# ybubnov/libhuffman

Hardware: AMD Instinct MI355X
Metric: encode+decode GiB/s (uncompressed) on 64KiB blocks (higher is better)
Workload: dtype u8; 1 GPU; configs[2]: 1 GiB Zipf-distributed bytes (zipf255 seed 3), blocksize=64KiB; generator=zipf255, bytes_per_gpu=1073741824, blocksize=65536, blocks_per_gpu=16384, compressed_bytes_per_gpu=1006904592, parallelism=block-sharded x1, bit_exact_roundtrip=True, decoder=sub-index (verified), one table pass per symbol

## Files before the change

libhuffman_amd/csrc/host/device.hpp:

```cpp
#pragma once

static SubStream sub_stream_args(const void *d_stream, uint64_t stream_len, const uint64_t *d_block_offsets, uint64_t nblocks,
                                 const void *d_sub_index, uint64_t raw_size, uint64_t blocksize, uint32_t flags)
{
    return {(const uint8_t *)d_stream, stream_len, d_block_offsets, nblocks, sub_index_view((void *)d_sub_index, raw_size, blocksize),
            raw_size, blocksize, max_tree_of(flags)};
}

extern "C" int hufgpu_fill(hufgpu_ctx_t *ctx, void *d_out, uint64_t n, int kind, uint64_t seed,
                           uint64_t first, void *stream)
{
    if (!ctx || (!d_out && n) || kind < 0 || kind > 3) return HUFE_ARGUMENT;
    if (n == 0) return HUFE_OK;
    if (kind == 1 && (first & 7)) {
        set_err(ctx, "uniform256 shards must start on an 8-byte boundary");
        return HUFE_ARGUMENT;
    }
    HIP_OK(ctx, hipSetDevice(ctx->device));
    hipStream_t s = pick_stream(ctx, stream);
    fill_kernel<<<dim3(4096), dim3(256), 0, s>>>((uint8_t *)d_out, n, kind, seed, first, ctx->d_zipf);
    HIP_OK(ctx, hipGetLastError());
    return HUFE_OK;
}

extern "C" int hufgpu_malloc(hufgpu_ctx_t *ctx, void **d_ptr, uint64_t bytes)
{
    if (!ctx || !d_ptr) return HUFE_ARGUMENT;
    HIP_OK(ctx, hipSetDevice(ctx->device));
    hipError_t e = hipMalloc(d_ptr, bytes ? bytes : 1);
    if (e != hipSuccess) {
        (void)hipGetLastError();
        set_err(ctx, "hipMalloc(%llu) failed: %s", (unsigned long long)bytes, hipGetErrorString(e));
        return HUFE_MEMORY;
    }
    return HUFE_OK;
}

extern "C" int hufgpu_free(hufgpu_ctx_t *ctx, void *d_ptr)
{
    if (!ctx) return HUFE_ARGUMENT;
    HIP_OK(ctx, hipSetDevice(ctx->device));
    HIP_OK(ctx, hipFree(d_ptr));
    return HUFE_OK;
}

extern "C" int hufgpu_memcpy_h2d(hufgpu_ctx_t *ctx, void *d_dst, const void *h_src, uint64_t bytes)
{
    if (!ctx) return HUFE_ARGUMENT;
    if (!bytes) return HUFE_OK;
    HIP_OK(ctx, hipSetDevice(ctx->device));
    HIP_OK(ctx, hipMemcpyAsync(d_dst, h_src, bytes, hipMemcpyHostToDevice, ctx->stream));
    HIP_OK(ctx, hipStreamSynchronize(ctx->stream));
    return HUFE_OK;
}

extern "C" int hufgpu_memcpy_d2h(hufgpu_ctx_t *ctx, void *h_dst, const void *d_src, uint64_t bytes)
{
    if (!ctx) return HUFE_ARGUMENT;
    if (!bytes) return HUFE_OK;
    HIP_OK(ctx, hipSetDevice(ctx->device));
    HIP_OK(ctx, hipMemcpyAsync(h_dst, d_src, bytes, hipMemcpyDeviceToHost, ctx->stream));
    HIP_OK(ctx, hipStreamSynchronize(ctx->stream));
    return HUFE_OK;
}

extern "C" int hufgpu_memcpy_d2d(hufgpu_ctx_t *ctx, void *d_dst, const void *d_src, uint64_t bytes)
{
    if (!ctx) return HUFE_ARGUMENT;
    if (!bytes) return HUFE_OK;
    HIP_OK(ctx, hipSetDevice(ctx->device));
    HIP_OK(ctx, hipMemcpyAsync(d_dst, d_src, bytes, hipMemcpyDeviceToDevice, ctx->stream));
    HIP_OK(ctx, hipStreamSynchronize(ctx->stream));
    return HUFE_OK;
}

extern "C" int hufgpu_synchronize(hufgpu_ctx_t *ctx)
{
    if (!ctx) return HUFE_ARGUMENT;
    HIP_OK(ctx, hipSetDevice(ctx->device));
    HIP_OK(ctx, hipStreamSynchronize(ctx->stream));
    return HUFE_OK;
}

template <int KIND>
static int calib_launch(int variant, const uint8_t *a, uint8_t *b, uint64_t bytes, uint32_t *flag, hipStream_t s)
{
#define CALIB_CASE(V, T, P, NTL, NTS) case V: calib_bw_kernel<T, P, KIND, NTL, NTS><<<dim3((unsigned)(bytes / P)), dim3(T), 0, s>>>(a, b, flag); return P;
    switch (variant) {
        CALIB_CASE(0, 256, 16384, true, true)
        CALIB_CASE(1, 256, 16384, true, false)
        CALIB_CASE(2, 256, 16384, false, false)
        CALIB_CASE(3, 512, 65536, true, true)
        CALIB_CASE(4, 512, 65536, true, false)
        CALIB_CASE(5, 256, 4096, true, true)
        CALIB_CASE(6, 256, 4096, false, false)
        CALIB_CASE(7, 1024, 65536, true, true)
    }
#undef CALIB_CASE
    return 0;
}
extern "C" int hufgpu_calib_bandwidth(hufgpu_ctx_t *ctx, int kind, int variant, const void *d_a, void *d_b, uint64_t bytes, void *stream)
{
    if (!ctx || kind < 0 || kind > 2 || variant < 0 || variant >= HUFGPU_CALIB_VARIANTS) return HUFE_ARGUMENT;
    if ((kind != 2 && !d_a) || (kind != 1 && !d_b) || bytes == 0 || (bytes & 65535u) || (((uintptr_t)d_a | (uintptr_t)d_b) & 15u)) return HUFE_ARGUMENT;
    HIP_OK(ctx, hipSetDevice(ctx->device));
    hipStream_t s = pick_stream(ctx, stream);
    uint32_t *flag = (uint32_t *)ctx->d_result;
    int per = 0;
    if (kind == 0) per = calib_launch<0>(variant, (const uint8_t *)d_a, (uint8_t *)d_b, bytes, flag + 6, s);
    else if (kind == 1) per = calib_launch<1>(variant, (const uint8_t *)d_a, (uint8_t *)d_b, bytes, flag + 6, s);
    else per = calib_launch<2>(variant, (const uint8_t *)d_a, (uint8_t *)d_b, bytes, flag + 6, s);
    HIP_OK(ctx, hipGetLastError());
    return per ? HUFE_OK : HUFE_ARGUMENT;
}

#ifdef DFAST_DEBUG
extern "C" int hufgpu_debug_dfast(unsigned long long *out32, int reset)
{
    if (reset) { unsigned long long z[DFAST_DBG_SLOTS] = {0}; return (int)hipMemcpyToSymbol(HIP_SYMBOL(hufgpu::g_dfast_dbg), z, sizeof(z)); }
    return (int)hipMemcpyFromSymbol(out32, HIP_SYMBOL(hufgpu::g_dfast_dbg), DFAST_DBG_SLOTS * sizeof(unsigned long long));
}
#endif
#ifdef TREE_DEBUG
extern "C" int hufgpu_debug_tree(unsigned long long *out, int reset)
{
    if (reset) { unsigned long long z[TREE_DBG_SLOTS] = {0}; return (int)hipMemcpyToSymbol(HIP_SYMBOL(hufgpu::g_tree_dbg), z, sizeof(z)); }
    return (int)hipMemcpyFromSymbol(out, HIP_SYMBOL(hufgpu::g_tree_dbg), TREE_DBG_SLOTS * sizeof(unsigned long long));
}
#endif

#ifdef DEC_PHASE_PROF
extern "C" int hufgpu_debug_phase_cycles(hufgpu_ctx_t *ctx, unsigned long long *out16, int reset)
{
    if (!ctx || !out16) return HUFE_ARGUMENT;
    HIP_OK(ctx, hipDeviceSynchronize());
    HIP_OK(ctx, hipMemcpyFromSymbol(out16, HIP_SYMBOL(hufgpu::g_dec_prof), 16 * sizeof(unsigned long long)));
    if (reset) {
        unsigned long long z[16] = {0};
        HIP_OK(ctx, hipMemcpyToSymbol(HIP_SYMBOL(hufgpu::g_dec_prof), z, sizeof(z)));
    }
    return HUFE_OK;
}
#endif
```

libhuffman_amd/csrc/kernels/pack.hpp:

```cpp
#pragma once
#include <hip/hip_runtime.h>
#include <stdint.h>

#include "../hufgpu_common.h"
#include "offsets.hpp"

namespace hufgpu {

#define PACK_SPT 32
#define PACK_STAGE_WORDS 3328

#define HUF_SUB_GROUP PACK_SPT
#define HUF_SUB_TILE  (64 * PACK_SPT)
struct HufSubIndex {
    uint64_t *tile_bits;
    uint16_t *group_bits;
    uint8_t *lens;
    uint64_t gpb, tpb;
};

template <typename CodeT>
struct PackAcc {
    uint64_t acc;
    uint32_t nacc;
    uint32_t first;
    bool have_first;
    uint32_t *gw;

    __device__ __forceinline__ void emit(uint32_t word)
    {
        if (!have_first) { first = word; have_first = true; }
        else *gw = __builtin_bswap32(word);
        gw++;
    }
    __device__ __forceinline__ void push32(uint32_t code, uint32_t len)
    {
        acc = (acc << len) | code;
        nacc += len;
        if (nacc >= 32) {
            nacc -= 32;
            emit((uint32_t)(acc >> nacc));
        }
    }
    __device__ __forceinline__ void push_pair(uint32_t e0, uint32_t e1)
    {
        const uint32_t l1 = e1 & 0xffu;
        push32(((e0 >> 8) << l1) | (e1 >> 8), (e0 & 0xffu) + l1);
    }
    __device__ __forceinline__ void push_triple(uint32_t e0, uint32_t e1, uint32_t e2)
    {
        const uint32_t l1 = e1 & 0xffu, l2 = e2 & 0xffu;
        push32(((((e0 >> 8) << l1) | (e1 >> 8)) << l2) | (e2 >> 8), (e0 & 0xffu) + l1 + l2);
    }
    __device__ __forceinline__ uint32_t tail() const { return (uint32_t)(acc & ((1ull << nacc) - 1ull)); }
    __device__ __forceinline__ void push(CodeT e)
    {
        uint32_t len = (uint32_t)(e & 0xffu);
        if constexpr (sizeof(CodeT) == 8) {
            const uint64_t c = e >> 8;
            if (len > 32) {
                push32((uint32_t)(c >> 32), len - 32);
                len = 32;
            }
            push32((uint32_t)c, len);
        } else {
            push32((uint32_t)(e >> 8), len);
        }
    }
};

#ifndef PACK_ACC64
template <>
struct PackAcc<uint32_t> {
    uint32_t acc;
    uint32_t nacc;
    uint32_t first;
    bool have_first;
    uint32_t *gw;

    __device__ __forceinline__ void emit(uint32_t word)
    {
        if (!have_first) { first = word; have_first = true; }
        else *gw = __builtin_bswap32(word);
        gw++;
    }
    __device__ __forceinline__ void push32(uint32_t code, uint32_t len)
    {
        const uint32_t out = acc >> ((32u - len) & 31u);
        acc = (acc << len) | code;
        nacc += len;
        if (nacc >= 32) {
            nacc -= 32;
            emit(__builtin_amdgcn_alignbit(out, acc, nacc));
        }
    }
    __device__ __forceinline__ void push_pair(uint32_t e0, uint32_t e1)
    {
        const uint32_t l1 = e1 & 0xffu;
        push32(((e0 >> 8) << l1) | (e1 >> 8), (e0 & 0xffu) + l1);
    }
    __device__ __forceinline__ void push_triple(uint32_t e0, uint32_t e1, uint32_t e2)
    {
        const uint32_t l1 = e1 & 0xffu, l2 = e2 & 0xffu;
        push32(((((e0 >> 8) << l1) | (e1 >> 8)) << l2) | (e2 >> 8), (e0 & 0xffu) + l1 + l2);
    }
    __device__ __forceinline__ void push(uint32_t e) { push32(e >> 8, e & 0xffu); }
    __device__ __forceinline__ uint32_t tail() const { return acc & ((1u << nacc) - 1u); }
};
#endif

__device__ __forceinline__ uint32_t header_byte(uint32_t j, uint64_t block_len, uint32_t tree_len,
                                                const int16_t *__restrict__ tb)
{
    if (j < 8) return (uint32_t)(block_len >> (8 * j)) & 0xffu;
    if (j < 10) return (tree_len >> (8 * (j - 8))) & 0xffu;
    const uint16_t e = (uint16_t)tb[(j - 10) >> 1];
    return (e >> (8 * (j & 1))) & 0xffu;
}

template <int THREADS>
__device__ __forceinline__ bool pack_header(uint64_t len, const int16_t *__restrict__ tb, uint32_t tree_len,
                                            uint8_t *g_a0, uint32_t *g_w0, uint32_t rec_lo, uint64_t rec_hi,
                                            uint32_t *s_tail, uint32_t *hdr_end_out)
{
    constexpr int WAVES = THREADS / 64;
    const int tid = (int)threadIdx.x;
    const uint32_t hdr_bytes = HUF_HEADER_FIXED + 2u * tree_len;
    const uint32_t hdr_end = rec_lo + hdr_bytes;
    for (uint32_t w = tid; w < (hdr_end >> 2); w += THREADS) {
        uint32_t v = 0;
#pragma unroll
        for (int k = 0; k < 4; k++) {
            const uint32_t bp = 4 * w + k;
            if (bp >= rec_lo) v |= header_byte(bp - rec_lo, len, tree_len, tb) << (8 * k);
        }
        if (4 * w >= rec_lo) g_w0[w] = v;
        else {
            for (uint32_t k = rec_lo - 4 * w; k < 4; k++) g_a0[4 * w + k] = (uint8_t)(v >> (8 * k));
        }
    }
    if (tree_len == 5) {
        for (uint32_t bp = (hdr_end & ~3u) + tid; bp < hdr_end; bp += THREADS)
            g_a0[bp] = (uint8_t)header_byte(bp - rec_lo, len, tree_len, tb);
        const uint64_t z0 = hdr_end, z1 = rec_hi;
        const uint64_t a0 = dmin<uint64_t>((z0 + 15) & ~15ull, z1);
        const uint64_t a1 = dmax<uint64_t>(a0, z1 & ~15ull);
        const uint64_t skew = (uint64_t)((uintptr_t)g_a0 & 15u);
        const uint64_t b0 = dmin<uint64_t>(((z0 + skew + 15) & ~15ull) - skew, z1);
        const uint64_t b1 = dmax<uint64_t>(b0, ((z1 + skew) & ~15ull) - skew);
        (void)a0; (void)a1;
        for (uint64_t bp = z0 + tid; bp < b0; bp += THREADS) g_a0[bp] = 0;
        uint4 *q = reinterpret_cast<uint4 *>(g_a0 + b0);
        const uint4 zero4 = make_uint4(0u, 0u, 0u, 0u);
        for (uint64_t i = (uint64_t)tid; i < ((b1 - b0) >> 4); i += THREADS) store_pack16(q + i, zero4);
        for (uint64_t bp = b1 + tid; bp < z1; bp += THREADS) g_a0[bp] = 0;
        return false;
    }
    if (tid == 0) {
        uint32_t t = 0;
        for (uint32_t bp = hdr_end & ~3u; bp < hdr_end; bp++)
            t = (t << 8) | header_byte(bp - rec_lo, len, tree_len, tb);
        s_tail[WAVES] = t;
    }
    __syncthreads();
    *hdr_end_out = hdr_end;
    return true;
}

template <int THREADS, typename CodeT, int GROUP = 1>
__device__ __forceinline__ void pack_block(const uint8_t *__restrict__ src, uint64_t len,
                                           const hufcode_t *__restrict__ codes64,
                                           const int16_t *__restrict__ tb, uint32_t tree_len,
                                           uint8_t *__restrict__ out, uint64_t dst0, uint64_t dst1,
                                           CodeT *s_code, uint32_t *s_part, uint32_t *s_tail, uint32_t *s_stage,
                                           uint64_t *__restrict__ sub_tiles, uint16_t *__restrict__ sub_groups)
{
    static_assert(HUF_SUB_TILE == 64 * PACK_SPT, "a sub-index tile is one wave of a pack tile");
    constexpr int TILE = THREADS * PACK_SPT;
    constexpr int WAVES = THREADS / 64;
    const int tid = (int)threadIdx.x;
    const int lane = tid & 63, wave = tid >> 6;

    uint8_t *g_a0 = out + (dst0 & ~3ull);
    const uint32_t rec_lo = (uint32_t)(dst0 & 3ull);
    const uint64_t rec_hi = rec_lo + (dst1 - dst0);
    uint32_t *g_w0 = reinterpret_cast<uint32_t *>(g_a0);

    for (int i = tid; i < HUF_NSYM; i += THREADS) s_code[i] = (CodeT)codes64[i];

    uint32_t hdr_end;
    if (!pack_header<THREADS>(len, tb, tree_len, g_a0, g_w0, rec_lo, rec_hi, s_tail, &hdr_end)) return;

    uint64_t bitpos = (uint64_t)hdr_end * 8ull;


    for (uint64_t t0 = 0; t0 < len; t0 += TILE) {
        const uint64_t my0 = t0 + (uint64_t)tid * PACK_SPT;
        uint32_t nsym = 0;
        CodeT code[PACK_SPT];
        uint32_t mybits = 0;
        if (my0 < len) {
            nsym = (uint32_t)dmin<uint64_t>(PACK_SPT, len - my0);
            const uint8_t *p = src + my0;
            if (nsym == PACK_SPT && (((uintptr_t)p) & 15u) == 0) {
                const uint4 v0 = load_stream16(reinterpret_cast<const uint4 *>(p));
                const uint4 v1 = load_stream16(reinterpret_cast<const uint4 *>(p) + 1);
                const uint32_t w[8] = {v0.x, v0.y, v0.z, v0.w, v1.x, v1.y, v1.z, v1.w};
#pragma unroll
                for (int k = 0; k < PACK_SPT; k++) code[k] = s_code[(w[k >> 2] >> (8 * (k & 3))) & 0xffu];
            } else {
#pragma unroll
                for (int k = 0; k < PACK_SPT; k++) code[k] = (k < (int)nsym) ? s_code[p[k]] : (CodeT)0;
            }
#pragma unroll
            for (int k = 0; k < PACK_SPT; k++) mybits += (uint32_t)(code[k] & 0xffu);
        } else {
#pragma unroll
            for (int k = 0; k < PACK_SPT; k++) code[k] = 0;
        }
        uint32_t tile_bits;
        const uint32_t ex = block_excl_scan_u32<THREADS>(mybits, s_part, tile_bits);
        if (sub_groups) {
            if (nsym) sub_groups[my0 / PACK_SPT] = (uint16_t)mybits;
            if (lane == 0 && nsym) sub_tiles[my0 / HUF_SUB_TILE] = bitpos + ex - (uint64_t)hdr_end * 8ull;
        }

        const uint64_t s = bitpos + ex;
        const uint64_t w_lo = bitpos >> 5, w_hi = (bitpos + tile_bits) >> 5;
        const uintptr_t stage_addr = (uintptr_t)(g_w0 + w_lo) & ~(uintptr_t)15;
        const uint32_t i_lo = (uint32_t)(((uintptr_t)(g_w0 + w_lo) - stage_addr) >> 2);
        const uint32_t i_hi = i_lo + (uint32_t)(w_hi - w_lo);
        const bool staged = i_hi + 2 <= PACK_STAGE_WORDS;
        PackAcc<CodeT> a;
        a.acc = 0;
        a.nacc = (uint32_t)(s & 31u);
        a.have_first = false;
        a.first = 0;
        uint32_t *const g_first = g_w0 + (s >> 5);
        uint32_t *const s_first = s_stage + (i_lo + (uint32_t)((s >> 5) - w_lo));
        if (staged) {
            a.gw = s_first;
            if constexpr (GROUP == 3) {
#pragma unroll
                for (int k = 0; k + 2 < PACK_SPT; k += 3) a.push_triple((uint32_t)code[k], (uint32_t)code[k + 1], (uint32_t)code[k + 2]);
                static_assert(PACK_SPT % 3 == 2, "the last two symbols go as a pair");
                a.push_pair((uint32_t)code[PACK_SPT - 2], (uint32_t)code[PACK_SPT - 1]);
            } else if constexpr (GROUP == 2) {
#pragma unroll
                for (int k = 0; k < PACK_SPT; k += 2) a.push_pair((uint32_t)code[k], (uint32_t)code[k + 1]);
            } else {
#pragma unroll
                for (int k = 0; k < PACK_SPT; k++) a.push(code[k]);
            }
        } else {
            a.gw = g_first;
#pragma unroll
            for (int k = 0; k < PACK_SPT; k++) a.push(code[k]);
        }
        const uint32_t nwords = (uint32_t)(a.gw - (staged ? s_first : g_first));
        const uint32_t tail_val = a.tail();

        uint32_t in_tail = wave_up1_u32(tail_val);
        if (lane == 63) s_tail[wave] = tail_val;
        __syncthreads();
        if (lane == 0) in_tail = (wave == 0) ? s_tail[WAVES] : s_tail[wave - 1];
        const uint32_t n_in = (uint32_t)(s & 31u);
        const bool is_last = (nsym > 0) && (my0 + nsym == len);
        if (a.have_first) {
            const uint32_t word = __builtin_bswap32(a.first | (n_in ? (in_tail << (32 - n_in)) : 0u));
            if (staged) *s_first = word;
            else *g_first = word;
        }
        uint32_t out_tail = tail_val;
        if (!a.have_first && nsym > 0) {
            out_tail = (n_in ? (in_tail << (a.nacc - n_in)) : 0u) | tail_val;
        }
        if (is_last && a.nacc) {
            const uint32_t word = out_tail << (32 - a.nacc);
            const uint32_t nbytes = (a.nacc + 7) >> 3;
            uint8_t *b = reinterpret_cast<uint8_t *>(g_first + nwords);
            for (uint32_t k = 0; k < nbytes; k++) b[k] = (uint8_t)(word >> (24 - 8 * k));
        }
        __syncthreads();
        if (tid == THREADS - 1) s_tail[WAVES] = out_tail;
        if (staged) {
            uint8_t *const g16 = reinterpret_cast<uint8_t *>(stage_addr);
            for (uint32_t u = tid; 4 * u < i_hi; u += THREADS) {
                const uint32_t i0 = 4 * u;
                if (i0 >= i_lo && i0 + 4 <= i_hi) {
                    store_pack16(reinterpret_cast<uint4 *>(g16 + 4 * i0), *reinterpret_cast<const uint4 *>(s_stage + i0));
                } else {
                    for (uint32_t i = (i0 > i_lo ? i0 : i_lo); i < i0 + 4 && i < i_hi; i++)
                        *reinterpret_cast<uint32_t *>(g16 + 4 * i) = s_stage[i];
                }
            }
        }
        bitpos += tile_bits;
        (void)rec_hi;
    }
}

struct PackEnt {
    uint32_t code;
    uint32_t lens;
};
__device__ __forceinline__ uint2 pack_ent_of(hufcode_t e)
{
    const uint32_t len = (uint32_t)(e & 0xffu);
    return make_uint2((uint32_t)(e >> 8), len | (((32u - len) & 31u) << 16) | (len << 27));
}
__device__ __forceinline__ uint32_t pack_pushed_out(uint32_t lens, uint32_t acc)
{
    uint32_t o;
    asm("v_lshrrev_b32_sdwa %0, %1, %2 dst_sel:DWORD dst_unused:UNUSED_PAD src0_sel:BYTE_2 src1_sel:DWORD"
        : "=v"(o) : "v"(lens), "v"(acc));
    return o;
}

template <int GROUP, bool PARTIAL>
__device__ __forceinline__ uint32_t pack_join(const uint2 *s_ent, const uint32_t (&w)[8], uint32_t nsym,
                                              uint32_t (&pc)[(PACK_SPT + GROUP - 1) / GROUP], uint32_t (&ph)[(PACK_SPT + GROUP - 1) / GROUP])
{
    constexpr int NG = (PACK_SPT + GROUP - 1) / GROUP;
    constexpr int BATCH = GROUP == 2 ? 4 : 2;
    uint32_t bits = 0;
#pragma unroll
    for (int g = 0; g < NG; g++) {
        if (g % BATCH == 0) __builtin_amdgcn_sched_barrier(0);
        const int k = g * GROUP;
        uint2 e[3];
#pragma unroll
        for (int j = 0; j < GROUP; j++) {
            const int kk = k + j;
            if (kk < PACK_SPT) {
                e[j] = s_ent[(w[kk >> 2] >> (8 * (kk & 3))) & 0xffu];
                if (PARTIAL && kk >= (int)nsym) e[j] = make_uint2(0u, 0u);
            }
        }
        if (GROUP == 3 && k + 2 < PACK_SPT) {
            pc[g] = (((e[0].x << (e[1].y & 31u)) | e[1].x) << (e[2].y & 31u)) | e[2].x;
            ph[g] = e[0].y + e[1].y + e[2].y;
        } else {
            pc[g] = (e[0].x << (e[1].y & 31u)) | e[1].x;
            ph[g] = e[0].y + e[1].y;
        }
        bits += ph[g];
    }
    __builtin_amdgcn_sched_barrier(0);
    return bits & 0xffffu;
}

template <int THREADS, int GROUP>
__device__ __forceinline__ void pack_block_multi(const uint8_t *__restrict__ src, uint64_t len64,
                                                 const hufcode_t *__restrict__ codes64,
                                                 const int16_t *__restrict__ tb, uint32_t tree_len,
                                                 uint8_t *__restrict__ out, uint64_t dst0, uint64_t dst1,
                                                 uint2 *s_ent, uint32_t *s_part, uint32_t *s_tail, uint32_t *s_stage,
                                                 uint64_t *__restrict__ sub_tiles, uint16_t *__restrict__ sub_groups)
{
    static_assert(GROUP == 2 || GROUP == 3, "two or three codes a push");
    static_assert(HUF_SUB_TILE == 64 * PACK_SPT, "a sub-index tile is one wave of a pack tile");
    constexpr uint32_t TILE = THREADS * PACK_SPT;
    constexpr int WAVES = THREADS / 64;
    const uint32_t len = (uint32_t)len64;
    constexpr int NG = (PACK_SPT + GROUP - 1) / GROUP;
    typedef __attribute__((address_space(3))) uint32_t *lds_word;
    const int tid = (int)threadIdx.x;
    const int lane = tid & 63, wave = tid >> 6;

    uint8_t *g_a0 = out + (dst0 & ~3ull);
    const uint32_t rec_lo = (uint32_t)(dst0 & 3ull);
    const uint64_t rec_hi = rec_lo + (dst1 - dst0);
    uint32_t *g_w0 = reinterpret_cast<uint32_t *>(g_a0);

    for (int i = tid; i < HUF_NSYM; i += THREADS) s_ent[i] = pack_ent_of(codes64[i]);

    uint32_t hdr_end;
    if (!pack_header<THREADS>(len64, tb, tree_len, g_a0, g_w0, rec_lo, rec_hi, s_tail, &hdr_end)) return;

    uint64_t bitpos = (uint64_t)hdr_end * 8ull;

    uint4 n0 = make_uint4(0u, 0u, 0u, 0u), n1 = n0;
    bool ahead = false;
#define PACK_REQUEST(T0_)                                                                                      \
    {                                                                                                         \
        const uint32_t m0_ = (T0_) + (uint32_t)tid * PACK_SPT;                                                \
        const uint8_t *q_ = src + m0_;                                                                        \
        ahead = (T0_) < len && __builtin_amdgcn_ballot_w64(!(m0_ + PACK_SPT <= len && (((uintptr_t)q_) & 15u) == 0)) == 0ull; \
        if (ahead) {                                                                                          \
            n0 = load_stream16(reinterpret_cast<const uint4 *>(q_));                                          \
            n1 = load_stream16(reinterpret_cast<const uint4 *>(q_) + 1);                                      \
        }                                                                                                     \
    }
    PACK_REQUEST(0u)
    for (uint32_t t0 = 0; t0 < len; t0 += TILE) {
        const uint32_t my0 = t0 + (uint32_t)tid * PACK_SPT;
        const uint32_t nsym = my0 < len ? dmin<uint32_t>(PACK_SPT, len - my0) : 0u;
        const uint8_t *p = src + my0;
        uint32_t pc[NG], ph[NG];
        uint32_t mybits;
        if (ahead) {
            const uint32_t w[8] = {n0.x, n0.y, n0.z, n0.w, n1.x, n1.y, n1.z, n1.w};
            mybits = pack_join<GROUP, false>(s_ent, w, nsym, pc, ph);
        } else {
            uint32_t w[8];
#pragma unroll
            for (int i = 0; i < 8; i++) {
                w[i] = 0;
#pragma unroll
                for (int j = 0; j < 4; j++)
                    if (4 * i + j < (int)nsym) w[i] |= (uint32_t)p[4 * i + j] << (8 * j);
            }
            mybits = pack_join<GROUP, true>(s_ent, w, nsym, pc, ph);
        }
        PACK_REQUEST(t0 + TILE)
        uint32_t tile_bits;
        const uint32_t ex = block_excl_scan_u32<THREADS>(mybits, s_part, tile_bits);
        if (sub_groups) {
            if (nsym) sub_groups[my0 / PACK_SPT] = (uint16_t)mybits;
            if (lane == 0 && nsym) sub_tiles[my0 / HUF_SUB_TILE] = bitpos + ex - (uint64_t)hdr_end * 8ull;
        }

        const uint64_t w_lo = bitpos >> 5, w_hi = (bitpos + tile_bits) >> 5;
        const uintptr_t stage_addr = (uintptr_t)(g_w0 + w_lo) & ~(uintptr_t)15;
        const uint32_t i_lo = (uint32_t)(((uintptr_t)(g_w0 + w_lo) - stage_addr) >> 2);
        const uint32_t i_hi = i_lo + (uint32_t)(w_hi - w_lo);
        const bool staged = i_hi + 2 <= PACK_STAGE_WORDS;
        const uint32_t rel = (uint32_t)(bitpos & 31u) + ex;
        const uint32_t n_in = rel & 31u;
        uint32_t *const g_first = g_w0 + w_lo + (rel >> 5);
        uint32_t *const s_first = s_stage + (i_lo + (rel >> 5));
        uint32_t nwords, nacc, tail_val, first = 0;
        if (staged) {
            uint32_t acc = 0;
            uint32_t tot = n_in | (n_in << 27);
            const uint32_t gw0 = (uint32_t)(uintptr_t)(lds_word)s_first - 4u;
            uint32_t gw = gw0;
#pragma unroll
            for (int g = 0; g < NG; g++) {
                uint32_t tot2;
                const bool word_done = __builtin_add_overflow(tot, ph[g], &tot2);
                const uint32_t acc2 = (acc << (ph[g] & 31u)) | pc[g];
                if (word_done) {
                    const uint32_t word = __builtin_amdgcn_alignbit(pack_pushed_out(ph[g], acc), acc2, tot2);
                    gw += 4;
                    asm volatile("" : "+v"(gw));
                    *(lds_word)(uintptr_t)gw = __builtin_bswap32(word);
                }
                acc = acc2;
                tot = tot2;
            }
            nwords = (gw - gw0) >> 2;
            nacc = tot & 31u;
            tail_val = acc & ((1u << nacc) - 1u);
        } else {
            PackAcc<uint32_t> a;
            a.acc = 0;
            a.nacc = n_in;
            a.have_first = false;
            a.first = 0;
            a.gw = g_first;
#pragma unroll 1
            for (uint32_t k = 0; k < nsym; k++) {
                const uint2 e = s_ent[src[my0 + k]];
                a.push32(e.x, e.y & 31u);
            }
            nwords = (uint32_t)(a.gw - g_first);
            nacc = a.nacc;
            tail_val = a.tail();
            first = a.first;
        }

        uint32_t in_tail = wave_up1_u32(tail_val);
        if (lane == 63) s_tail[wave] = tail_val;
        __syncthreads();
        if (lane == 0) in_tail = (wave == 0) ? s_tail[WAVES] : s_tail[wave - 1];
        const bool is_last = (nsym > 0) && (my0 + nsym == len);
        if (nwords) {
            const uint32_t lead = n_in ? (in_tail << (32 - n_in)) : 0u;
            if (staged) {
                if (n_in) __hip_atomic_fetch_or(s_first, __builtin_bswap32(lead), __ATOMIC_RELAXED, __HIP_MEMORY_SCOPE_WORKGROUP);
            } else {
                *g_first = __builtin_bswap32(first | lead);
            }
        }
        uint32_t out_tail = tail_val;
        if (!nwords && nsym > 0) {
            out_tail = (n_in ? (in_tail << (nacc - n_in)) : 0u) | tail_val;
        }
        if (is_last && nacc) {
            const uint32_t word = out_tail << (32 - nacc);
            const uint32_t nbytes = (nacc + 7) >> 3;
            uint8_t *b = reinterpret_cast<uint8_t *>(g_first + nwords);
            for (uint32_t k = 0; k < nbytes; k++) b[k] = (uint8_t)(word >> (24 - 8 * k));
        }
        __syncthreads();
        if (tid == THREADS - 1) s_tail[WAVES] = out_tail;
        if (staged) {
            uint8_t *const g16 = reinterpret_cast<uint8_t *>(stage_addr);
            for (uint32_t u = tid; 4 * u < i_hi; u += THREADS) {
                const uint32_t i0 = 4 * u;
                if (i0 >= i_lo && i0 + 4 <= i_hi) {
                    store_pack16(reinterpret_cast<uint4 *>(g16 + 4 * i0), *reinterpret_cast<const uint4 *>(s_stage + i0));
                } else {
                    for (uint32_t i = (i0 > i_lo ? i0 : i_lo); i < i0 + 4 && i < i_hi; i++)
                        *reinterpret_cast<uint32_t *>(g16 + 4 * i) = s_stage[i];
                }
            }
        }
        bitpos += tile_bits;
        (void)rec_hi;
    }
}

#undef PACK_REQUEST

template <int THREADS, bool SHORT>
__device__ __forceinline__ void pack_block_any(const uint8_t *__restrict__ src, uint64_t len, uint64_t row, uint64_t blk,
                                               const hufcode_t *__restrict__ codetab,
                                               const int16_t *__restrict__ treebuf,
                                               const HufBlockMeta *__restrict__ meta,
                                               uint64_t *__restrict__ offsets, const TwoLevel &sizes,
                                               uint8_t *__restrict__ out, const HufSubIndex &sub,
                                               hufcode_t *s_code, uint32_t *s_part, uint32_t *s_tail, uint32_t *s_stage)
{
    const HufBlockMeta m = meta[row];
    const hufcode_t *codes = codetab + row * HUF_NSYM;
    const int16_t *tb = treebuf + row * HUF_TREE_STRIDE;
    uint64_t o0, o1;
    if (sizes.local) {
        o0 = sizes.gprefix[blk / SCAN_GROUP] + sizes.local[blk];
        o1 = o0 + encoded_block_bytes(m);
        if (threadIdx.x == 0) offsets[blk] = o0;
    } else {
        o0 = offsets[blk];
        o1 = offsets[blk + 1];
    }
    uint64_t *sub_tiles = sub.tile_bits ? sub.tile_bits + blk * sub.tpb : nullptr;
    uint16_t *sub_groups = sub.tile_bits ? sub.group_bits + blk * sub.gpb : nullptr;
    if (sub.tile_bits && m.tree_len != 5)
        for (int i = (int)threadIdx.x; i < HUF_NSYM; i += THREADS) sub.lens[blk * HUF_NSYM + i] = (uint8_t)(codes[i] & 0xffu);
#if !defined(PACK_ACC64)
    if (m.max_len <= 10)
        pack_block_multi<THREADS, 3>(src, len, codes, tb, m.tree_len, out, o0, o1,
                                     reinterpret_cast<uint2 *>(s_code), s_part, s_tail, s_stage, sub_tiles, sub_groups);
    else if (m.max_len <= 15)
        pack_block_multi<THREADS, 2>(src, len, codes, tb, m.tree_len, out, o0, o1,
                                     reinterpret_cast<uint2 *>(s_code), s_part, s_tail, s_stage, sub_tiles, sub_groups);
#else
    if (m.max_len <= 10)
        pack_block<THREADS, uint32_t, 3>(src, len, codes, tb, m.tree_len, out, o0, o1,
                                         reinterpret_cast<uint32_t *>(s_code), s_part, s_tail, s_stage, sub_tiles, sub_groups);
    else if (m.max_len <= 15)
        pack_block<THREADS, uint32_t, 2>(src, len, codes, tb, m.tree_len, out, o0, o1,
                                            reinterpret_cast<uint32_t *>(s_code), s_part, s_tail, s_stage, sub_tiles, sub_groups);
#endif
    else if (SHORT || m.max_len <= 24)
        pack_block<THREADS, uint32_t>(src, len, codes, tb, m.tree_len, out, o0, o1,
                                      reinterpret_cast<uint32_t *>(s_code), s_part, s_tail, s_stage, sub_tiles, sub_groups);
    else if constexpr (!SHORT)
        pack_block<THREADS, hufcode_t>(src, len, codes, tb, m.tree_len, out, o0, o1,
                                       s_code, s_part, s_tail, s_stage, sub_tiles, sub_groups);
}

template <int THREADS, bool SHORT>
__device__ __forceinline__ void pack_block_any(const uint8_t *__restrict__ src, uint64_t len, uint64_t blk,
                                               const hufcode_t *__restrict__ codetab,
                                               const int16_t *__restrict__ treebuf,
                                               const HufBlockMeta *__restrict__ meta,
                                               uint64_t *__restrict__ offsets, const TwoLevel &sizes,
                                               uint8_t *__restrict__ out, const HufSubIndex &sub,
                                               hufcode_t *s_code, uint32_t *s_part, uint32_t *s_tail, uint32_t *s_stage)
{
    pack_block_any<THREADS, SHORT>(src, len, blk, blk, codetab, treebuf, meta, offsets, sizes, out, sub, s_code, s_part, s_tail, s_stage);
}

#ifndef PACK_WAVES_PER_SIMD
#define PACK_WAVES_PER_SIMD 6
#endif
template <int THREADS, bool SHORT>
__global__ __launch_bounds__(THREADS, SHORT ? PACK_WAVES_PER_SIMD : 4) void pack_kernel(const uint8_t *__restrict__ in, uint64_t n,
                                                       uint64_t blocksize,
                                                       const hufcode_t *__restrict__ codetab,
                                                       const int16_t *__restrict__ treebuf,
                                                       const HufBlockMeta *__restrict__ meta,
                                                       uint64_t *__restrict__ offsets, TwoLevel sizes,
                                                       uint8_t *__restrict__ out, HufSubIndex sub)
{
    __shared__ hufcode_t s_code[HUF_NSYM];
    __shared__ uint32_t s_part[THREADS / 64];
    __shared__ uint32_t s_tail[THREADS / 64 + 1];
    __shared__ __attribute__((aligned(16))) uint32_t s_stage[PACK_STAGE_WORDS];

#ifdef PACK_VGPR_SLACK
    asm volatile("; one VGPR more than the kernel uses" ::: PACK_VGPR_SLACK);
#endif
    const uint64_t blk = blockIdx.x;
    const uint64_t base = blk * blocksize;
    const uint64_t len = dmin<uint64_t>(blocksize, n - base);
    pack_block_any<THREADS, SHORT>(in + base, len, blk, codetab, treebuf, meta, offsets, sizes, out, sub,
                                   s_code, s_part, s_tail, s_stage);
}

}
```

libhuffman_amd/csrc/kernels/util.hpp:

```cpp
#pragma once
#include <hip/hip_runtime.h>
#include <stdint.h>

#include "../hufgpu_common.h"

namespace hufgpu {

__device__ __forceinline__ int lane_id() { return (int)(threadIdx.x & 63u); }

__device__ __forceinline__ uint32_t uni32(uint32_t v) { return (uint32_t)__builtin_amdgcn_readfirstlane((int)v); }
__device__ __forceinline__ uint64_t uni64(uint64_t v)
{
    return ((uint64_t)uni32((uint32_t)(v >> 32)) << 32) | uni32((uint32_t)v);
}
__device__ __forceinline__ void pin_uniform(uint64_t v)
{
    asm volatile("" :: "s"((uint32_t)v), "s"((uint32_t)(v >> 32)));
}

template <typename T>
__device__ __forceinline__ T dmin(T a, T b) { return a < b ? a : b; }
template <typename T>
__device__ __forceinline__ T dmax(T a, T b) { return a > b ? a : b; }

__device__ __forceinline__ uint64_t encoded_block_bytes(const HufBlockMeta &m)
{
    return (uint64_t)HUF_HEADER_FIXED + 2ull * m.tree_len + ((m.payload_bits + 7) >> 3);
}

__device__ __forceinline__ uint4 load_stream16(const uint4 *p)
{
    typedef uint32_t v4u __attribute__((ext_vector_type(4)));
    const v4u v = __builtin_nontemporal_load(reinterpret_cast<const v4u *>(p));
    return make_uint4(v.x, v.y, v.z, v.w);
}
__device__ __forceinline__ void store_stream16(uint4 *p, uint4 v)
{
    typedef uint32_t v4u __attribute__((ext_vector_type(4)));
    v4u t; t.x = v.x; t.y = v.y; t.z = v.z; t.w = v.w;
    __builtin_nontemporal_store(t, reinterpret_cast<v4u *>(p));
}
__device__ __forceinline__ void store_pack16(uint4 *p, uint4 v)
{
    *p = v;
}

__device__ __forceinline__ uint32_t wave_xor_any(uint32_t v, int o);
__device__ __forceinline__ uint64_t shfl_xor_u64(uint64_t v, int mask)
{
    return ((uint64_t)wave_xor_any((uint32_t)(v >> 32), mask) << 32) | wave_xor_any((uint32_t)v, mask);
}
__device__ __forceinline__ uint32_t shfl_xor_key(uint32_t v, int mask) { return (uint32_t)__shfl_xor((int)v, mask); }
__device__ __forceinline__ uint64_t shfl_xor_key(uint64_t v, int mask) { return shfl_xor_u64(v, mask); }

__device__ __forceinline__ uint32_t wave_incl_scan_u32(uint32_t v)
{
    v += (uint32_t)__builtin_amdgcn_update_dpp(0, (int)v, 0x111, 0xf, 0xf, true);
    v += (uint32_t)__builtin_amdgcn_update_dpp(0, (int)v, 0x112, 0xf, 0xf, true);
    v += (uint32_t)__builtin_amdgcn_update_dpp(0, (int)v, 0x114, 0xf, 0xf, true);
    v += (uint32_t)__builtin_amdgcn_update_dpp(0, (int)v, 0x118, 0xf, 0xf, true);
    v += (uint32_t)__builtin_amdgcn_update_dpp(0, (int)v, 0x142, 0xa, 0xf, false);
    v += (uint32_t)__builtin_amdgcn_update_dpp(0, (int)v, 0x143, 0xc, 0xf, false);
    return v;
}
__device__ __forceinline__ uint32_t wave_excl_max_u32(uint32_t v)
{
#define HUF_MAX_DPP_(ctrl, rmask, bc) { const uint32_t o_ = (uint32_t)__builtin_amdgcn_update_dpp(0, (int)v, ctrl, rmask, 0xf, bc); v = v > o_ ? v : o_; }
    HUF_MAX_DPP_(0x111, 0xf, true)
    HUF_MAX_DPP_(0x112, 0xf, true)
    HUF_MAX_DPP_(0x114, 0xf, true)
    HUF_MAX_DPP_(0x118, 0xf, true)
    HUF_MAX_DPP_(0x142, 0xa, false)
    HUF_MAX_DPP_(0x143, 0xc, false)
#undef HUF_MAX_DPP_
    return (uint32_t)__builtin_amdgcn_update_dpp(0, (int)v, 0x138, 0xf, 0xf, true);
}
__device__ __forceinline__ uint32_t pk_max_u16(uint32_t a, uint32_t b)
{
    typedef unsigned short us2 __attribute__((ext_vector_type(2)));
    const us2 r = __builtin_elementwise_max(__builtin_bit_cast(us2, a), __builtin_bit_cast(us2, b));
    return __builtin_bit_cast(uint32_t, r);
}

template <int D>
__device__ __forceinline__ uint32_t wave_xor_u32(uint32_t v)
{
    if constexpr (D == 1) return (uint32_t)__builtin_amdgcn_update_dpp(0, (int)v, 0xB1, 0xf, 0xf, false);
    else if constexpr (D == 2) return (uint32_t)__builtin_amdgcn_update_dpp(0, (int)v, 0x4E, 0xf, 0xf, false);
    else if constexpr (D == 4) {
        const uint32_t a = (uint32_t)__builtin_amdgcn_update_dpp(0, (int)v, 0x124, 0xf, 0xf, false);
        const uint32_t b = (uint32_t)__builtin_amdgcn_update_dpp(0, (int)v, 0x12C, 0xf, 0xf, false);
        return (lane_id() & 4) ? a : b;
    } else if constexpr (D == 8) return (uint32_t)__builtin_amdgcn_update_dpp(0, (int)v, 0x128, 0xf, 0xf, false);
    else if constexpr (D == 16) return (uint32_t)__builtin_amdgcn_ds_swizzle((int)v, 0x401F);
    else return (uint32_t)__shfl_xor((int)v, D);
}

__device__ __forceinline__ uint32_t wave_xor_any(uint32_t v, int o)
{
    return o == 1 ? wave_xor_u32<1>(v) : o == 2 ? wave_xor_u32<2>(v) : o == 4 ? wave_xor_u32<4>(v)
         : o == 8 ? wave_xor_u32<8>(v) : o == 16 ? wave_xor_u32<16>(v) : wave_xor_u32<32>(v);
}
__device__ __forceinline__ uint32_t wave_up1_u32(uint32_t v)
{
    return (uint32_t)__builtin_amdgcn_update_dpp((int)v, (int)v, 0x138, 0xf, 0xf, false);
}

__device__ __forceinline__ uint32_t wave_lane_u32(uint32_t v, uint32_t uniform_lane)
{
    return (uint32_t)__builtin_amdgcn_readlane((int)v, (int)uniform_lane);
}

template <int THREADS>
__device__ __forceinline__ uint32_t block_excl_scan_u32(uint32_t v, uint32_t *s_part, uint32_t &total)
{
    const int lane = lane_id();
    const int wave = (int)(threadIdx.x >> 6);
    const uint32_t inc = wave_incl_scan_u32(v);
    if (lane == 63) s_part[wave] = inc;
    __syncthreads();
    uint32_t base = 0, tot = 0;
#pragma unroll
    for (int i = 0; i < THREADS / 64; i++) {
        const uint32_t x = s_part[i];
        if (i < wave) base += x;
        tot += x;
    }
    __syncthreads();
    total = tot;
    return base + inc - v;
}

template <int THREADS, typename T>
__device__ __forceinline__ T block_excl_scan(T v, T *s_part, T &total)
{
    const int lane = lane_id();
    const int wave = (int)(threadIdx.x >> 6);
    T inc = v;
#pragma unroll
    for (int o = 1; o < 64; o <<= 1) {
        T t;
        if constexpr (sizeof(T) == 8) {
            uint32_t lo = (uint32_t)inc, hi = (uint32_t)((uint64_t)inc >> 32);
            lo = (uint32_t)__shfl_up((int)lo, o);
            hi = (uint32_t)__shfl_up((int)hi, o);
            t = (T)(((uint64_t)hi << 32) | lo);
        } else {
            t = (T)__shfl_up((int)inc, o);
        }
        if (lane >= o) inc += t;
    }
    if (lane == 63) s_part[wave] = inc;
    __syncthreads();
    T base = 0, tot = 0;
#pragma unroll
    for (int i = 0; i < THREADS / 64; i++) {
        T x = s_part[i];
        if (i < wave) base += x;
        tot += x;
    }
    __syncthreads();
    total = tot;
    return base + inc - v;
}

}
```

Baseline: 878.0 GiB/s.

## Overlap pack prologue loads: batch metadata scalar loads, prefetch codes/tree, vectorize header

Restructures the encode pack prologue. Per-block metadata and offsets are fetched with grouped scalar loads behind a single wait. Each thread loads its code-table entry and tree dwords up front, and the first input tile is requested before the header is written. The header is then built from registers with alignbit word stores instead of byte-wise loops, and the lens-row write is folded into the same pass. This aims to cut serialized memory latency at block start; the cost is more complex rec_lo alignment logic. It also adds optional cycle-profiling hooks that are compiled out by default.

```diff
diff --git a/libhuffman_amd/csrc/host/device.hpp b/libhuffman_amd/csrc/host/device.hpp
--- a/libhuffman_amd/csrc/host/device.hpp
+++ b/libhuffman_amd/csrc/host/device.hpp
@@ -129,6 +129,20 @@
 }
 #endif
 
+#ifdef PACK_PHASE_PROF
+extern "C" int hufgpu_debug_pack_phase_cycles(hufgpu_ctx_t *ctx, unsigned long long *out16, int reset)
+{
+    if (!ctx || !out16) return HUFE_ARGUMENT;
+    HIP_OK(ctx, hipDeviceSynchronize());
+    HIP_OK(ctx, hipMemcpyFromSymbol(out16, HIP_SYMBOL(hufgpu::g_pack_prof), 16 * sizeof(unsigned long long)));
+    if (reset) {
+        unsigned long long z[16] = {0};
+        HIP_OK(ctx, hipMemcpyToSymbol(HIP_SYMBOL(hufgpu::g_pack_prof), z, sizeof(z)));
+    }
+    return HUFE_OK;
+}
+#endif
+
 #ifdef DEC_PHASE_PROF
 extern "C" int hufgpu_debug_phase_cycles(hufgpu_ctx_t *ctx, unsigned long long *out16, int reset)
 {
diff --git a/libhuffman_amd/csrc/kernels/pack.hpp b/libhuffman_amd/csrc/kernels/pack.hpp
--- a/libhuffman_amd/csrc/kernels/pack.hpp
+++ b/libhuffman_amd/csrc/kernels/pack.hpp
@@ -118,37 +118,88 @@
     return (e >> (8 * (j & 1))) & 0xffu;
 }
 
+#ifdef PACK_PHASE_PROF
+__device__ unsigned long long g_pack_prof[16];
+#define PPROF_T() (__builtin_readcyclecounter())
+#define PPROF_ADD(slot, t0) do { if (threadIdx.x == 0) atomicAdd(&g_pack_prof[slot], (unsigned long long)(__builtin_readcyclecounter() - (t0))); } while (0)
+#define PPROF_WAIT() asm volatile("s_waitcnt vmcnt(0)" ::: "memory")
+#else
+#define PPROF_T() 0ull
+#define PPROF_ADD(slot, t0) do { (void)(t0); } while (0)
+#define PPROF_WAIT() do { } while (0)
+#endif
+
+#define PACK_TREE_DWORDS (HUF_TREE_STRIDE / 2)
+struct PackPre {
+    hufcode_t code;
+    uint32_t t[4];
+};
 template <int THREADS>
-__device__ __forceinline__ bool pack_header(uint64_t len, const int16_t *__restrict__ tb, uint32_t tree_len,
+__device__ __forceinline__ PackPre pack_pre_request(const hufcode_t *__restrict__ codes64, const int16_t *__restrict__ tb, uint32_t tid)
+{
+    static_assert(THREADS == HUF_NSYM, "one code-table entry a thread");
+    static_assert(3 * THREADS >= PACK_TREE_DWORDS && HUF_TREE_STRIDE % 4 == 0, "three tree dwords a thread cover an aligned row");
+    static_assert(2 * HUF_TREE_MAX <= 4 * (PACK_TREE_DWORDS - 1), "the look-ahead dword of the tree's last bytes is inside the row");
+    const uint32_t *tw = reinterpret_cast<const uint32_t *>(tb);
+    PackPre p;
+    p.code = codes64[tid];
+#pragma unroll
+    for (uint32_t k = 0; k < 4; k++) p.t[k] = tw[dmin<uint32_t>(3u * tid + k, PACK_TREE_DWORDS - 1u)];
+    return p;
+}
+
+__device__ __forceinline__ void pack_pre_arrived(const PackPre &p)
+{
+    asm volatile("" :: "v"((uint32_t)p.code), "v"((uint32_t)(p.code >> 32)), "v"(p.t[0]), "v"(p.t[1]), "v"(p.t[2]), "v"(p.t[3]));
+    __builtin_amdgcn_sched_barrier(0);
+}
+
+template <int THREADS>
+__device__ __forceinline__ bool pack_header(uint64_t len, const PackPre &pre, uint32_t tree_len,
                                             uint8_t *g_a0, uint32_t *g_w0, uint32_t rec_lo, uint64_t rec_hi,
-                                            uint32_t *s_tail, uint32_t *hdr_end_out)
+                                            uint32_t *s_tail, uint32_t *hdr_end_out, uint32_t tid)
 {
     constexpr int WAVES = THREADS / 64;
-    const int tid = (int)threadIdx.x;
     const uint32_t hdr_bytes = HUF_HEADER_FIXED + 2u * tree_len;
     const uint32_t hdr_end = rec_lo + hdr_bytes;
-    for (uint32_t w = tid; w < (hdr_end >> 2); w += THREADS) {
-        uint32_t v = 0;
-#pragma unroll
-        for (int k = 0; k < 4; k++) {
-            const uint32_t bp = 4 * w + k;
-            if (bp >= rec_lo) v |= header_byte(bp - rec_lo, len, tree_len, tb) << (8 * k);
-        }
-        if (4 * w >= rec_lo) g_w0[w] = v;
+    const uint32_t nwhole = hdr_end >> 2, nb = hdr_end & 3u;
+    const uint32_t wq0 = 3u + (rec_lo == 3u ? 1u : 0u);
+    const uint32_t cut = (8u * (2u - rec_lo)) & 31u;
+    if (tid == 0) {
+        const uint32_t f[4] = {(uint32_t)len, (uint32_t)(len >> 32), (tree_len & 0xffffu) | (pre.t[0] << 16), (pre.t[0] >> 16) | (pre.t[1] << 16)};
+        const uint32_t up = (32u - 8u * rec_lo) & 31u;
+        uint32_t v[4];
+        v[0] = f[0] << (8u * rec_lo);
+#pragma unroll
+        for (int w = 1; w < 4; w++) v[w] = rec_lo ? __builtin_amdgcn_alignbit(f[w], f[w - 1], up) : f[w];
+        if (rec_lo == 0) g_w0[0] = v[0];
         else {
-            for (uint32_t k = rec_lo - 4 * w; k < 4; k++) g_a0[4 * w + k] = (uint8_t)(v >> (8 * k));
+#pragma unroll
+            for (uint32_t k = 1; k < 4; k++)
+                if (k >= rec_lo) g_a0[k] = (uint8_t)(v[0] >> (8 * k));
+        }
+        g_w0[1] = v[1];
+        g_w0[2] = v[2];
+        if (rec_lo == 3) g_w0[3] = v[3];
+    }
+#pragma unroll
+    for (uint32_t k = 0; k < 3; k++) {
+        const uint32_t w = 3u * tid + k + wq0;
+        const uint32_t v = __builtin_amdgcn_alignbit(pre.t[k + 1], pre.t[k], cut);
+        if (w < nwhole) g_w0[w] = v;
+        else if (w == nwhole) {
+            if (tree_len == 5) {
+                for (uint32_t j = 0; j < nb; j++) g_a0[4 * w + j] = (uint8_t)(v >> (8 * j));
+            } else {
+                s_tail[WAVES] = nb ? __builtin_bswap32(v) >> (32u - 8u * nb) : 0u;
+            }
         }
     }
     if (tree_len == 5) {
-        for (uint32_t bp = (hdr_end & ~3u) + tid; bp < hdr_end; bp += THREADS)
-            g_a0[bp] = (uint8_t)header_byte(bp - rec_lo, len, tree_len, tb);
         const uint64_t z0 = hdr_end, z1 = rec_hi;
-        const uint64_t a0 = dmin<uint64_t>((z0 + 15) & ~15ull, z1);
-        const uint64_t a1 = dmax<uint64_t>(a0, z1 & ~15ull);
         const uint64_t skew = (uint64_t)((uintptr_t)g_a0 & 15u);
         const uint64_t b0 = dmin<uint64_t>(((z0 + skew + 15) & ~15ull) - skew, z1);
         const uint64_t b1 = dmax<uint64_t>(b0, ((z1 + skew) & ~15ull) - skew);
-        (void)a0; (void)a1;
         for (uint64_t bp = z0 + tid; bp < b0; bp += THREADS) g_a0[bp] = 0;
         uint4 *q = reinterpret_cast<uint4 *>(g_a0 + b0);
         const uint4 zero4 = make_uint4(0u, 0u, 0u, 0u);
@@ -156,12 +207,6 @@
         for (uint64_t bp = b1 + tid; bp < z1; bp += THREADS) g_a0[bp] = 0;
         return false;
     }
-    if (tid == 0) {
-        uint32_t t = 0;
-        for (uint32_t bp = hdr_end & ~3u; bp < hdr_end; bp++)
-            t = (t << 8) | header_byte(bp - rec_lo, len, tree_len, tb);
-        s_tail[WAVES] = t;
-    }
     __syncthreads();
     *hdr_end_out = hdr_end;
     return true;
@@ -173,12 +218,14 @@
                                            const int16_t *__restrict__ tb, uint32_t tree_len,
                                            uint8_t *__restrict__ out, uint64_t dst0, uint64_t dst1,
                                            CodeT *s_code, uint32_t *s_part, uint32_t *s_tail, uint32_t *s_stage,
-                                           uint64_t *__restrict__ sub_tiles, uint16_t *__restrict__ sub_groups)
+                                           uint64_t *__restrict__ sub_tiles, uint16_t *__restrict__ sub_groups, uint8_t *__restrict__ lens_row)
 {
     static_assert(HUF_SUB_TILE == 64 * PACK_SPT, "a sub-index tile is one wave of a pack tile");
     constexpr int TILE = THREADS * PACK_SPT;
     constexpr int WAVES = THREADS / 64;
-    const int tid = (int)threadIdx.x;
+    int tid = (int)threadIdx.x;
+    asm volatile("" : "+v"(tid));
+    __builtin_assume(tid >= 0 && tid < THREADS);
     const int lane = tid & 63, wave = tid >> 6;
 
     uint8_t *g_a0 = out + (dst0 & ~3ull);
@@ -186,16 +233,19 @@
     const uint64_t rec_hi = rec_lo + (dst1 - dst0);
     uint32_t *g_w0 = reinterpret_cast<uint32_t *>(g_a0);
 
-    for (int i = tid; i < HUF_NSYM; i += THREADS) s_code[i] = (CodeT)codes64[i];
+    const PackPre pre = pack_pre_request<THREADS>(codes64, tb, (uint32_t)tid);
+    pack_pre_arrived(pre);
+    s_code[tid] = (CodeT)pre.code;
+    if (lens_row) lens_row[tid] = (uint8_t)(pre.code & 0xffu);
 
     uint32_t hdr_end;
-    if (!pack_header<THREADS>(len, tb, tree_len, g_a0, g_w0, rec_lo, rec_hi, s_tail, &hdr_end)) return;
+    if (!pack_header<THREADS>(len, pre, tree_len, g_a0, g_w0, rec_lo, rec_hi, s_tail, &hdr_end, (uint32_t)tid)) return;
 
     uint64_t bitpos = (uint64_t)hdr_end * 8ull;
 
 
     for (uint64_t t0 = 0; t0 < len; t0 += TILE) {
-        const uint64_t my0 = t0 + (uint64_t)tid * PACK_SPT;
+        const uint64_t my0 = t0 + (uint64_t)((uint32_t)tid * PACK_SPT);
         uint32_t nsym = 0;
         CodeT code[PACK_SPT];
         uint32_t mybits = 0;
@@ -284,7 +334,7 @@
         __syncthreads();
         if (tid == THREADS - 1) s_tail[WAVES] = out_tail;
         if (staged) {
-            uint8_t *const g16 = reinterpret_cast<uint8_t *>(stage_addr);
+            uint8_t *const g16 = reinterpret_cast<uint8_t *>(g_w0 + ((int64_t)w_lo - (int64_t)i_lo));
             for (uint32_t u = tid; 4 * u < i_hi; u += THREADS) {
                 const uint32_t i0 = 4 * u;
                 if (i0 >= i_lo && i0 + 4 <= i_hi) {
@@ -350,13 +400,26 @@
     return bits & 0xffffu;
 }
 
+__device__ __forceinline__ bool pack_request(const uint8_t *__restrict__ src, uint32_t len, uint32_t t0, uint32_t tid, uint4 &n0, uint4 &n1)
+{
+    const uint32_t m0 = t0 + tid * PACK_SPT;
+    const uint8_t *q = src + m0;
+    const bool ahead = t0 < len && __builtin_amdgcn_ballot_w64(!(m0 + PACK_SPT <= len && (((uintptr_t)q) & 15u) == 0)) == 0ull;
+    if (ahead) {
+        n0 = load_stream16(reinterpret_cast<const uint4 *>(q));
+        n1 = load_stream16(reinterpret_cast<const uint4 *>(q) + 1);
+    }
+    return ahead;
+}
+
 template <int THREADS, int GROUP>
 __device__ __forceinline__ void pack_block_multi(const uint8_t *__restrict__ src, uint64_t len64,
                                                  const hufcode_t *__restrict__ codes64,
                                                  const int16_t *__restrict__ tb, uint32_t tree_len,
                                                  uint8_t *__restrict__ out, uint64_t dst0, uint64_t dst1,
                                                  uint2 *s_ent, uint32_t *s_part, uint32_t *s_tail, uint32_t *s_stage,
-                                                 uint64_t *__restrict__ sub_tiles, uint16_t *__restrict__ sub_groups)
+                                                 uint64_t *__restrict__ sub_tiles, uint16_t *__restrict__ sub_groups, uint8_t *__restrict__ lens_row,
+                                                 unsigned long long t_entry)
 {
     static_assert(GROUP == 2 || GROUP == 3, "two or three codes a push");
     static_assert(HUF_SUB_TILE == 64 * PACK_SPT, "a sub-index tile is one wave of a pack tile");
@@ -365,7 +428,9 @@
     const uint32_t len = (uint32_t)len64;
     constexpr int NG = (PACK_SPT + GROUP - 1) / GROUP;
     typedef __attribute__((address_space(3))) uint32_t *lds_word;
-    const int tid = (int)threadIdx.x;
+    int tid = (int)threadIdx.x;
+    asm volatile("" : "+v"(tid));
+    __builtin_assume(tid >= 0 && tid < THREADS);
     const int lane = tid & 63, wave = tid >> 6;
 
     uint8_t *g_a0 = out + (dst0 & ~3ull);
@@ -373,32 +438,41 @@
     const uint64_t rec_hi = rec_lo + (dst1 - dst0);
     uint32_t *g_w0 = reinterpret_cast<uint32_t *>(g_a0);
 
-    for (int i = tid; i < HUF_NSYM; i += THREADS) s_ent[i] = pack_ent_of(codes64[i]);
-
-    uint32_t hdr_end;
-    if (!pack_header<THREADS>(len64, tb, tree_len, g_a0, g_w0, rec_lo, rec_hi, s_tail, &hdr_end)) return;
-
-    uint64_t bitpos = (uint64_t)hdr_end * 8ull;
-
+    const PackPre pre = pack_pre_request<THREADS>(codes64, tb, (uint32_t)tid);
     uint4 n0 = make_uint4(0u, 0u, 0u, 0u), n1 = n0;
     bool ahead = false;
-#define PACK_REQUEST(T0_)                                                                                      \
-    {                                                                                                         \
-        const uint32_t m0_ = (T0_) + (uint32_t)tid * PACK_SPT;                                                \
-        const uint8_t *q_ = src + m0_;                                                                        \
-        ahead = (T0_) < len && __builtin_amdgcn_ballot_w64(!(m0_ + PACK_SPT <= len && (((uintptr_t)q_) & 15u) == 0)) == 0ull; \
-        if (ahead) {                                                                                          \
-            n0 = load_stream16(reinterpret_cast<const uint4 *>(q_));                                          \
-            n1 = load_stream16(reinterpret_cast<const uint4 *>(q_) + 1);                                      \
-        }                                                                                                     \
-    }
-    PACK_REQUEST(0u)
+#define PACK_REQUEST(T0_) { ahead = pack_request(src, len, (T0_), (uint32_t)tid, n0, n1); }
+    {
+        const uint8_t *q = src + (uint32_t)tid * PACK_SPT;
+        ahead = tree_len != 5 && 0u < len &&
+                __builtin_amdgcn_ballot_w64(!((uint32_t)tid * PACK_SPT + PACK_SPT <= len && (((uintptr_t)q) & 15u) == 0)) == 0ull;
+        const uint4 *q16 = ahead ? reinterpret_cast<const uint4 *>(q) : reinterpret_cast<const uint4 *>(codes64);
+        n0 = load_stream16(q16);
+        n1 = load_stream16(q16 + 1);
+    }
+    pack_pre_arrived(pre);
+    s_ent[tid] = pack_ent_of(pre.code);
+    if (lens_row) lens_row[tid] = (uint8_t)(pre.code & 0xffu);
+
+    uint32_t hdr_end;
+    if (!pack_header<THREADS>(len64, pre, tree_len, g_a0, g_w0, rec_lo, rec_hi, s_tail, &hdr_end, (uint32_t)tid)) return;
+    PPROF_ADD(0, t_entry);
+    unsigned long long pt = PPROF_T();
+
+    uint64_t bitpos = (uint64_t)hdr_end * 8ull;
+    bool first_tile = true;
+    (void)first_tile;
     for (uint32_t t0 = 0; t0 < len; t0 += TILE) {
         const uint32_t my0 = t0 + (uint32_t)tid * PACK_SPT;
         const uint32_t nsym = my0 < len ? dmin<uint32_t>(PACK_SPT, len - my0) : 0u;
         const uint8_t *p = src + my0;
         uint32_t pc[NG], ph[NG];
         uint32_t mybits;
+#ifdef PACK_PHASE_PROF
+        if (first_tile) { PPROF_ADD(1, pt); first_tile = false; pt = PPROF_T(); }
+        PPROF_WAIT();
+        PPROF_ADD(2, pt); pt = PPROF_T();
+#endif
         if (ahead) {
             const uint32_t w[8] = {n0.x, n0.y, n0.z, n0.w, n1.x, n1.y, n1.z, n1.w};
             mybits = pack_join<GROUP, false>(s_ent, w, nsym, pc, ph);
@@ -414,12 +488,14 @@
             mybits = pack_join<GROUP, true>(s_ent, w, nsym, pc, ph);
         }
         PACK_REQUEST(t0 + TILE)
+        PPROF_ADD(3, pt); pt = PPROF_T();
         uint32_t tile_bits;
         const uint32_t ex = block_excl_scan_u32<THREADS>(mybits, s_part, tile_bits);
         if (sub_groups) {
             if (nsym) sub_groups[my0 / PACK_SPT] = (uint16_t)mybits;
             if (lane == 0 && nsym) sub_tiles[my0 / HUF_SUB_TILE] = bitpos + ex - (uint64_t)hdr_end * 8ull;
         }
+        PPROF_ADD(4, pt); pt = PPROF_T();
 
         const uint64_t w_lo = bitpos >> 5, w_hi = (bitpos + tile_bits) >> 5;
         const uintptr_t stage_addr = (uintptr_t)(g_w0 + w_lo) & ~(uintptr_t)15;
@@ -495,9 +571,10 @@
             for (uint32_t k = 0; k < nbytes; k++) b[k] = (uint8_t)(word >> (24 - 8 * k));
         }
         __syncthreads();
+        PPROF_ADD(5, pt); pt = PPROF_T();
         if (tid == THREADS - 1) s_tail[WAVES] = out_tail;
         if (staged) {
-            uint8_t *const g16 = reinterpret_cast<uint8_t *>(stage_addr);
+            uint8_t *const g16 = reinterpret_cast<uint8_t *>(g_w0 + ((int64_t)w_lo - (int64_t)i_lo));
             for (uint32_t u = tid; 4 * u < i_hi; u += THREADS) {
                 const uint32_t i0 = 4 * u;
                 if (i0 >= i_lo && i0 + 4 <= i_hi) {
@@ -510,7 +587,9 @@
         }
         bitpos += tile_bits;
         (void)rec_hi;
-    }
+        PPROF_ADD(6, pt); pt = PPROF_T();
+    }
+    PPROF_ADD(7, t_entry);
 }
 
 #undef PACK_REQUEST
@@ -524,43 +603,50 @@
                                                uint8_t *__restrict__ out, const HufSubIndex &sub,
                                                hufcode_t *s_code, uint32_t *s_part, uint32_t *s_tail, uint32_t *s_stage)
 {
-    const HufBlockMeta m = meta[row];
+    const unsigned long long t_entry = PPROF_T();
     const hufcode_t *codes = codetab + row * HUF_NSYM;
     const int16_t *tb = treebuf + row * HUF_TREE_STRIDE;
+    HufBlockMeta m;
     uint64_t o0, o1;
     if (sizes.local) {
-        o0 = sizes.gprefix[blk / SCAN_GROUP] + sizes.local[blk];
+        uint64_t gp, lc;
+        const uint4 mw = sload_4_2_2(meta + row, sizes.gprefix + blk / SCAN_GROUP, sizes.local + blk, gp, lc);
+        m.tree_len = mw.x; m.max_len = mw.y; m.payload_bits = ((uint64_t)mw.w << 32) | mw.z;
+        o0 = gp + lc;
         o1 = o0 + encoded_block_bytes(m);
         if (threadIdx.x == 0) offsets[blk] = o0;
     } else {
-        o0 = offsets[blk];
-        o1 = offsets[blk + 1];
+        uint4 ow;
+        const uint4 mw = sload_4_4(meta + row, offsets + blk, ow);
+        m.tree_len = mw.x; m.max_len = mw.y; m.payload_bits = ((uint64_t)mw.w << 32) | mw.z;
+        o0 = ((uint64_t)ow.y << 32) | ow.x;
+        o1 = ((uint64_t)ow.w << 32) | ow.z;
     }
     uint64_t *sub_tiles = sub.tile_bits ? sub.tile_bits + blk * sub.tpb : nullptr;
     uint16_t *sub_groups = sub.tile_bits ? sub.group_bits + blk * sub.gpb : nullptr;
-    if (sub.tile_bits && m.tree_len != 5)
-        for (int i = (int)threadIdx.x; i < HUF_NSYM; i += THREADS) sub.lens[blk * HUF_NSYM + i] = (uint8_t)(codes[i] & 0xffu);
+    uint8_t *lens_row = (sub.tile_bits && m.tree_len != 5) ? sub.lens + blk * HUF_NSYM : nullptr;
 #if !defined(PACK_ACC64)
     if (m.max_len <= 10)
         pack_block_multi<THREADS, 3>(src, len, codes, tb, m.tree_len, out, o0, o1,
-                                     reinterpret_cast<uint2 *>(s_code), s_part, s_tail, s_stage, sub_tiles, sub_groups);
+                                     reinterpret_cast<uint2 *>(s_code), s_part, s_tail, s_stage, sub_tiles, sub_groups, lens_row, t_entry);
     else if (m.max_len <= 15)
         pack_block_multi<THREADS, 2>(src, len, codes, tb, m.tree_len, out, o0, o1,
-                                     reinterpret_cast<uint2 *>(s_code), s_part, s_tail, s_stage, sub_tiles, sub_groups);
+                                     reinterpret_cast<uint2 *>(s_code), s_part, s_tail, s_stage, sub_tiles, sub_groups, lens_row, t_entry);
 #else
     if (m.max_len <= 10)
         pack_block<THREADS, uint32_t, 3>(src, len, codes, tb, m.tree_len, out, o0, o1,
-                                         reinterpret_cast<uint32_t *>(s_code), s_part, s_tail, s_stage, sub_tiles, sub_groups);
+                                         reinterpret_cast<uint32_t *>(s_code), s_part, s_tail, s_stage, sub_tiles, sub_groups, lens_row);
     else if (m.max_len <= 15)
         pack_block<THREADS, uint32_t, 2>(src, len, codes, tb, m.tree_len, out, o0, o1,
-                                            reinterpret_cast<uint32_t *>(s_code), s_part, s_tail, s_stage, sub_tiles, sub_groups);
+                                            reinterpret_cast<uint32_t *>(s_code), s_part, s_tail, s_stage, sub_tiles, sub_groups, lens_row);
 #endif
     else if (SHORT || m.max_len <= 24)
         pack_block<THREADS, uint32_t>(src, len, codes, tb, m.tree_len, out, o0, o1,
-                                      reinterpret_cast<uint32_t *>(s_code), s_part, s_tail, s_stage, sub_tiles, sub_groups);
+                                      reinterpret_cast<uint32_t *>(s_code), s_part, s_tail, s_stage, sub_tiles, sub_groups, lens_row);
     else if constexpr (!SHORT)
         pack_block<THREADS, hufcode_t>(src, len, codes, tb, m.tree_len, out, o0, o1,
-                                       s_code, s_part, s_tail, s_stage, sub_tiles, sub_groups);
+                                       s_code, s_part, s_tail, s_stage, sub_tiles, sub_groups, lens_row);
+    (void)t_entry;
 }
 
 template <int THREADS, bool SHORT>
diff --git a/libhuffman_amd/csrc/kernels/util.hpp b/libhuffman_amd/csrc/kernels/util.hpp
--- a/libhuffman_amd/csrc/kernels/util.hpp
+++ b/libhuffman_amd/csrc/kernels/util.hpp
@@ -16,6 +16,24 @@
 __device__ __forceinline__ void pin_uniform(uint64_t v)
 {
     asm volatile("" :: "s"((uint32_t)v), "s"((uint32_t)(v >> 32)));
+}
+
+__device__ __forceinline__ uint4 sload_4_2_2(const void *a4, const void *b2, const void *c2, uint64_t &vb, uint64_t &vc)
+{
+    typedef uint32_t v4u __attribute__((ext_vector_type(4)));
+    v4u va;
+    asm volatile("s_load_dwordx4 %0, %3, 0x0\n\ts_load_dwordx2 %1, %4, 0x0\n\ts_load_dwordx2 %2, %5, 0x0\n\ts_waitcnt lgkmcnt(0)"
+                 : "=&s"(va), "=&s"(vb), "=&s"(vc) : "s"(a4), "s"(b2), "s"(c2));
+    return make_uint4(va.x, va.y, va.z, va.w);
+}
+__device__ __forceinline__ uint4 sload_4_4(const void *a4, const void *b4, uint4 &vb)
+{
+    typedef uint32_t v4u __attribute__((ext_vector_type(4)));
+    v4u va, wb;
+    asm volatile("s_load_dwordx4 %0, %2, 0x0\n\ts_load_dwordx4 %1, %3, 0x0\n\ts_waitcnt lgkmcnt(0)"
+                 : "=&s"(va), "=&s"(wb) : "s"(a4), "s"(b4));
+    vb = make_uint4(wb.x, wb.y, wb.z, wb.w);
+    return make_uint4(va.x, va.y, va.z, va.w);
 }
 
 template <typename T>
```

New measurement: 888.0 GiB/s (median of 6 runs). Within noise of the previous version (+1.1%).
